# aharley/pips

Hardware: AMD Instinct MI355X
Metric: particle-updates/sec (B*S*N*iters/s) at S=8 N=256 368x496 (higher is better)
Workload: dtype f32; 1 GPU; BASELINE configs[1]: B=1/GPU S=8 368x496 N=256 I=6 fp32 stride 8, encoder included, inputs resident in HBM; clips_per_gpu=1, parallelism=clip-sharded x1, collective=none

## Files before the change

pips_amd/csrc/conv_f32_r.hip:

```cpp
#include "common.h"

namespace pips {

constexpr int CR_ROWS = 4, CR_COLS = 32, CR_TN = 32, CR_PITCH = 272;
constexpr int CR_PW = CR_COLS + 2, CR_PH = CR_ROWS + 2;
constexpr int CR_WBYTES = 9 * CR_TN * CR_PITCH, CR_PBYTES = CR_PH * CR_PW * CR_PITCH;
constexpr int CR_LDS = CR_WBYTES + CR_PBYTES;
constexpr int CR_NCH = CR_PH * CR_PW * 16, CR_NIT = (CR_NCH + 255) / 256;
constexpr unsigned CR_OOB = 0x80000000u;

struct ConvRArgs {
    const float* in; const float* wgt; const float* bias; float* out; float* stats; const float* in_norm;
    int H, W, tiles_x, tiles, bph;
    int by_xcd;
};

typedef unsigned u32x4 __attribute__((ext_vector_type(4)));

__global__ __launch_bounds__(256) void conv3x3_c64_f32_r_kernel(ConvRArgs p) {
    extern __shared__ __attribute__((aligned(16))) char smem[];
    char* Wl = smem;
    char* Pl = smem + CR_WBYTES;
    const int tid = threadIdx.x, lane = tid & 63;
    const int wave = __builtin_amdgcn_readfirstlane(tid >> 6);
    const int l31 = lane & 31, half = lane >> 5;
    const int H = p.H, W = p.W;
    int f, rem;
    if (p.by_xcd) {
        const int per = 16 * p.bph, grp = blockIdx.x / per, j = blockIdx.x - grp * per;
        f = 8 * grp + (j & 7); rem = j >> 3;
    } else {
        f = blockIdx.x / (2 * p.bph); rem = blockIdx.x - f * (2 * p.bph);
    }
    const int hc = rem & 1, b = rem >> 1;

    {
        constexpr int NW = 9 * CR_TN * 16 / 256;
        float4 wv[NW];
#pragma unroll
        for (int k = 0; k < NW; ++k) {
            const int i = tid + 256 * k, row = i >> 4, tap = row >> 5, co = row & 31;
            wv[k] = *reinterpret_cast<const float4*>(p.wgt + ((size_t)(hc * CR_TN + co) * 9 + tap) * 64 + (i & 15) * 4);
        }
#pragma unroll
        for (int k = 0; k < NW; ++k) {
            const int i = tid + 256 * k;
            *reinterpret_cast<float4*>(Wl + (i >> 4) * CR_PITCH + (i & 15) * 16) = wv[k];
        }
    }

    const __amdgpu_buffer_rsrc_t rsrc = __builtin_amdgcn_make_buffer_rsrc(
        const_cast<float*>(p.in + (size_t)f * H * W * 64), (short)0, (int)((unsigned)(H * W) * 256u), 0x00020000);
    const int chunk = tid & 15;
    unsigned goff[CR_NIT], pyx[CR_NIT];
#pragma unroll
    for (int it = 0; it < CR_NIT; ++it) {
        const int pix = (tid >> 4) + it * 16;
        const int py = pix / CR_PW, px = pix - py * CR_PW;
        goff[it] = (unsigned)((py * W + px) * 256 + chunk * 16);
        pyx[it] = (unsigned)(py | px << 8);
    }
    const bool last_ok = tid + (CR_NIT - 1) * 256 < CR_NCH;
    char* lds_dst = Pl + (tid >> 4) * CR_PITCH + chunk * 16;
    float4 nrm[2] = {make_float4(0.f, 1.f, 0.f, 1.f), make_float4(0.f, 1.f, 0.f, 1.f)};
    if (p.in_norm != nullptr) {
        const float4* np = reinterpret_cast<const float4*>(p.in_norm + ((size_t)f * 64 + chunk * 4) * 2);
        nrm[0] = np[0]; nrm[1] = np[1];
    }

    u32x4 fr[CR_NIT];
    unsigned inside = 0;
    auto fetch = [&](int t, bool live) __attribute__((always_inline)) {
        const int ty = t / p.tiles_x, tx = t - ty * p.tiles_x;
        const int y0 = ty * CR_ROWS, x0 = tx * CR_COLS;
        const unsigned base = (unsigned)(((y0 - 1) * W + (x0 - 1)) * 256);
        const bool interior = y0 >= 1 && y0 + CR_ROWS + 1 <= H && x0 >= 1 && x0 + CR_COLS + 1 <= W;
        if (interior) {
            inside = last_ok ? (1u << CR_NIT) - 1 : (1u << (CR_NIT - 1)) - 1;
#pragma unroll
            for (int it = 0; it < CR_NIT; ++it) {
                const unsigned off = (live && (it + 1 < CR_NIT || last_ok)) ? base + goff[it] : CR_OOB;
                fr[it] = __builtin_amdgcn_raw_buffer_load_b128(rsrc, (int)off, 0, 0);
            }
        } else {
            inside = 0;
#pragma unroll
            for (int it = 0; it < CR_NIT; ++it) {
                const int gy = y0 - 1 + (int)(pyx[it] & 0xff), gx = x0 - 1 + (int)(pyx[it] >> 8);
                const bool ok = live && (it + 1 < CR_NIT || last_ok) && (unsigned)gy < (unsigned)H && (unsigned)gx < (unsigned)W;
                inside |= ok ? 1u << it : 0u;
                fr[it] = __builtin_amdgcn_raw_buffer_load_b128(rsrc, (int)(ok ? base + goff[it] : CR_OOB), 0, 0);
            }
        }
    };
    auto stage = [&]() __attribute__((always_inline)) {
#pragma unroll
        for (int it = 0; it < CR_NIT; ++it) {
            if (it + 1 < CR_NIT || last_ok) {
                float4 v = make_float4(__uint_as_float(fr[it].x), __uint_as_float(fr[it].y), __uint_as_float(fr[it].z),
                                       __uint_as_float(fr[it].w));
                if (p.in_norm != nullptr) {
                    const bool in = inside >> it & 1;
                    const float nx = fmaxf((v.x - nrm[0].x) * nrm[0].y, 0.f), ny = fmaxf((v.y - nrm[0].z) * nrm[0].w, 0.f);
                    const float nz = fmaxf((v.z - nrm[1].x) * nrm[1].y, 0.f), nw = fmaxf((v.w - nrm[1].z) * nrm[1].w, 0.f);
                    v = make_float4(in ? nx : 0.f, in ? ny : 0.f, in ? nz : 0.f, in ? nw : 0.f);
                }
                *reinterpret_cast<float4*>(lds_dst + it * (16 * CR_PITCH)) = v;
            }
        }
    };

    const int col = hc * CR_TN + l31;
    const float bv = p.bias[col];
    const char* pa = Pl + (wave * CR_PW + l31) * CR_PITCH + half * 16;
    const char* pb = Wl + l31 * CR_PITCH + half * 16;
    const int parts = p.tiles * 4;
    const __amdgpu_buffer_rsrc_t rsrc_out = __builtin_amdgcn_make_buffer_rsrc(
        p.out + (size_t)f * H * W * 64, (short)0, (int)((unsigned)(H * W) * 256u), 0x00020000);
    const __amdgpu_buffer_rsrc_t rsrc_st = __builtin_amdgcn_make_buffer_rsrc(
        p.stats + (size_t)f * parts * 256, (short)0, (int)((unsigned)parts * 1024u), 0x00020000);

    float bvs = bv;
    asm volatile("" : "+v"(bvs), "+v"(nrm[0].x), "+v"(nrm[0].y), "+v"(nrm[0].z), "+v"(nrm[0].w), "+v"(nrm[1].x), "+v"(nrm[1].y),
                 "+v"(nrm[1].z), "+v"(nrm[1].w));
    fetch(b, true);
#pragma unroll
    for (int r = 0; r < 16; ++r) __builtin_amdgcn_raw_buffer_store_b32((unsigned)r, rsrc_out, (int)(CR_OOB + 256u * r), 0, 0);
    __builtin_amdgcn_raw_buffer_store_b128((u32x4){0u, 0u, 0u, 0u}, rsrc_st, (int)CR_OOB, 0, 0);
    for (int t = b; t < p.tiles; t += p.bph) {
        lds_barrier();
        stage();
        lds_barrier();
        fetch(t + p.bph < p.tiles ? t + p.bph : t, t + p.bph < p.tiles);
        __builtin_amdgcn_sched_barrier(0);

        f32x16 acc;
#pragma unroll
        for (int r = 0; r < 16; ++r) acc[r] = 0.f;
        constexpr int CR_AHEAD = 2, CR_NBUF = 3;
        float4 fa[CR_NBUF], fb[CR_NBUF];
#define PIPS_CR_LOAD(g_)                                                                                                \
        {                                                                                                               \
            constexpr int tap_ = (g_) / 8, kb_ = (g_) % 8, kh_ = tap_ / 3, kw_ = tap_ % 3, buf_ = (g_) % CR_NBUF;         \
            fa[buf_] = *reinterpret_cast<const float4*>(pa + (kh_ * CR_PW + kw_) * CR_PITCH + kb_ * 32);                 \
            fb[buf_] = *reinterpret_cast<const float4*>(pb + tap_ * (CR_TN * CR_PITCH) + kb_ * 32);                      \
        }
#define PIPS_CR_STEP(g_)                                                                                                \
        if constexpr ((g_) + CR_AHEAD < 72) PIPS_CR_LOAD((g_) + CR_AHEAD)                                               \
        acc = __builtin_amdgcn_mfma_f32_32x32x2f32(fa[(g_) % CR_NBUF].x, fb[(g_) % CR_NBUF].x, acc, 0, 0, 0);            \
        acc = __builtin_amdgcn_mfma_f32_32x32x2f32(fa[(g_) % CR_NBUF].y, fb[(g_) % CR_NBUF].y, acc, 0, 0, 0);            \
        acc = __builtin_amdgcn_mfma_f32_32x32x2f32(fa[(g_) % CR_NBUF].z, fb[(g_) % CR_NBUF].z, acc, 0, 0, 0);            \
        acc = __builtin_amdgcn_mfma_f32_32x32x2f32(fa[(g_) % CR_NBUF].w, fb[(g_) % CR_NBUF].w, acc, 0, 0, 0);            \
        __builtin_amdgcn_sched_barrier(0);
#define PIPS_CR_STEP8(g_)                                                                                               \
        PIPS_CR_STEP(g_) PIPS_CR_STEP((g_) + 1) PIPS_CR_STEP((g_) + 2) PIPS_CR_STEP((g_) + 3) PIPS_CR_STEP((g_) + 4)      \
        PIPS_CR_STEP((g_) + 5) PIPS_CR_STEP((g_) + 6) PIPS_CR_STEP((g_) + 7)
        PIPS_CR_LOAD(0) PIPS_CR_LOAD(1)
        __builtin_amdgcn_sched_barrier(0);
        PIPS_CR_STEP8(0) PIPS_CR_STEP8(8) PIPS_CR_STEP8(16) PIPS_CR_STEP8(24) PIPS_CR_STEP8(32) PIPS_CR_STEP8(40) PIPS_CR_STEP8(48)
        PIPS_CR_STEP8(56) PIPS_CR_STEP8(64)
#undef PIPS_CR_STEP8
#undef PIPS_CR_STEP
#undef PIPS_CR_LOAD

        const int ty = t / p.tiles_x, tx = t - ty * p.tiles_x;
        const int y = ty * CR_ROWS + wave, x0 = tx * CR_COLS;
        const int nvalid = y < H ? min(CR_COLS, W - x0) : 0;
        const unsigned obase = (unsigned)(((y * W + x0) * 64 + col) * 4);
        const float piv1 = __shfl(acc[1] + bvs, l31), piv0 = __shfl(acc[0] + bvs, l31);
        const float pivot = nvalid > 1 ? piv1 : piv0;
        float cs = 0.f, cq = 0.f;
#pragma unroll
        for (int r = 0; r < 16; ++r) {
            const int px = (r & 3) + 8 * (r >> 2) + 4 * half;
            const float v = acc[r] + bvs;
            const bool ok = px < nvalid;
            __builtin_amdgcn_raw_buffer_store_b32(__float_as_uint(v), rsrc_out, (int)(ok ? obase + (unsigned)px * 256u : CR_OOB), 0, 0);
            const float d = ok ? v - pivot : 0.f;
            cs += d;
            cq += d * d;
        }
        const float s1 = cs + __shfl_xor(cs, 32), s2 = cq + __shfl_xor(cq, 32);
        const u32x4 sv = {__float_as_uint(s1), __float_as_uint(s2), __float_as_uint(pivot), __float_as_uint((float)nvalid)};
        __builtin_amdgcn_raw_buffer_store_b128(sv, rsrc_st, (int)(half == 0 ? (unsigned)(((t * 4 + wave) * 64 + col) * 16) : CR_OOB), 0, 0);
    }
}

bool conv_f32_r_admits(const GemmArgs& a) {
    if (a.KH != 3 || a.KW != 3 || a.cstride != 1 || a.pad != 1 || a.Cin != 64 || a.N != 64 || a.ldc != 64 || a.Ho != a.H ||
        a.Wo != a.Win || a.bias == nullptr || a.stats == nullptr)
        return false;
    if ((unsigned long long)(a.H + 2) * (a.Win + 2) * 256ull >= (1ull << 31)) return false;
    const long parts = 4l * cdiv(a.H, CR_ROWS) * cdiv(a.Win, CR_COLS);
    const long cap = a.stats_parts_cap > 0 ? a.stats_parts_cap : 2 * cdiv(a.M, 64) + 4;
    return parts <= cap && parts * 64 * 16 < (1l << 31);
}

bool conv_f32_r_takes(const GemmArgs& a, int frames) {
    if (!PIPS_TUNE("PIPS_CONV_F32_R", 1) || !conv_f32_r_admits(a)) return false;
    const int cus = device_cus();
    const long tiles = 2l * cdiv(a.H, CR_ROWS) * cdiv(a.Win, CR_COLS) * frames;
    return cus > 0 && tiles * 100 >= (long)cus * PIPS_TUNE("PIPS_CONV_F32_R_MINPCT", 300);
}

int launch_conv_f32_r(const GemmArgs& a, int frames, int* parts_out, hipStream_t st) {
    const int cus = device_cus();
    if (cus <= 0) {
        set_error("conv3x3_c64_f32_r: cannot query the device");
        return PIPS_E_LAUNCH;
    }
    static std::atomic<unsigned long long> raised{0};
    const int rc = ensure_dynamic_lds(raised, (const void*)conv3x3_c64_f32_r_kernel, CR_LDS);
    if (rc != PIPS_OK) return rc;
    ConvRArgs p;
    p.in = a.A; p.wgt = a.W; p.bias = a.bias; p.out = a.C; p.stats = a.stats; p.in_norm = a.in_norm;
    p.H = a.H; p.W = a.Win; p.tiles_x = cdiv(a.Win, CR_COLS); p.tiles = p.tiles_x * cdiv(a.H, CR_ROWS);
    p.bph = max(1, min(p.tiles, cdiv(cus, 2 * frames)));
    p.by_xcd = (frames % 8 == 0) && PIPS_TUNE("PIPS_CONV_F32_R_XCD", 1);
    hipLaunchKernelGGL(conv3x3_c64_f32_r_kernel, dim3(frames * 2 * p.bph), dim3(256), CR_LDS, st, p);
    PIPS_CHECK_LAUNCH("conv3x3_c64_f32_r_kernel");
    if (parts_out) *parts_out = p.tiles * 4;
    return PIPS_OK;
}

}
```

Baseline: 1.410 million particle-updates/s.

## Compute two 4-row halves per weight fetch with XOR-swizzled unpadded LDS

The 3x3 conv tile grows from 4 to up to 8 output rows per work item. Each wave now keeps two MFMA accumulators that share the same weight fragment loads, so B-operand LDS traffic per output drops. The padded LDS pitch is replaced by an XOR swizzle on 16-byte chunks to avoid bank conflicts. Next-tile global loads are interleaved into the MFMA k-loop instead of being issued in one burst, and work is split into contiguous unit ranges per block. The staging path gets specialized normalization variants. An optional timing trace is compiled in only under a macro. The trade-offs are higher register pressure from the doubled accumulators and more index bookkeeping.

Result: no change. 1.409 million particle-updates/s (-0.1%).

```diff
diff --git a/pips_amd/csrc/conv_f32_r.hip b/pips_amd/csrc/conv_f32_r.hip
--- a/pips_amd/csrc/conv_f32_r.hip
+++ b/pips_amd/csrc/conv_f32_r.hip
@@ -1,26 +1,78 @@
+#include <type_traits>
+
 #include "common.h"
 
 namespace pips {
 
-constexpr int CR_ROWS = 4, CR_COLS = 32, CR_TN = 32, CR_PITCH = 272;
-constexpr int CR_PW = CR_COLS + 2, CR_PH = CR_ROWS + 2;
-constexpr int CR_WBYTES = 9 * CR_TN * CR_PITCH, CR_PBYTES = CR_PH * CR_PW * CR_PITCH;
+constexpr int CR_HROWS = 4, CR_COLS = 32, CR_TN = 32, CR_ROWB = 256;
+constexpr int CR_PW = CR_COLS + 2, CR_PH = 2 * CR_HROWS + 2;
+constexpr int CR_WBYTES = 9 * CR_TN * CR_ROWB, CR_PBYTES = CR_PH * CR_PW * CR_ROWB;
 constexpr int CR_LDS = CR_WBYTES + CR_PBYTES;
 constexpr int CR_NCH = CR_PH * CR_PW * 16, CR_NIT = (CR_NCH + 255) / 256;
 constexpr unsigned CR_OOB = 0x80000000u;
+static_assert(CR_LDS <= 163840, "conv3x3_c64_f32_r: weights and patch must fit the compute unit's LDS");
 
 struct ConvRArgs {
     const float* in; const float* wgt; const float* bias; float* out; float* stats; const float* in_norm;
-    int H, W, tiles_x, tiles, bph;
+    int H, W, tiles_x, rows4;
+    int units, ufull, bph;
     int by_xcd;
 };
 
 typedef unsigned u32x4 __attribute__((ext_vector_type(4)));
 
+#ifdef PIPS_CONV_R_TRACE
+__device__ unsigned long long* g_cr_trace = nullptr;
+#define PIPS_CR_T(i_)                                                        \
+    {                                                                        \
+        __builtin_amdgcn_sched_barrier(0);                                   \
+        const unsigned long long now_ = __builtin_amdgcn_s_memtime();        \
+        tr_acc[i_] += now_ - tr_last;                                        \
+        tr_last = now_;                                                      \
+        __builtin_amdgcn_sched_barrier(0);                                   \
+    }
+#else
+#define PIPS_CR_T(i_)
+#endif
+
+template <int NCH>
+__device__ __forceinline__ void cr_kloop(const char* smem, const unsigned (&pa)[3][8], const unsigned (&pb)[8], f32x16& acc0, f32x16& acc1,
+                                         const __amdgpu_buffer_rsrc_t rsrc, const unsigned (&poff)[CR_NIT], u32x4 (&fr)[CR_NIT]) {
+    static_assert(3 * (CR_NIT - 1) + 1 < 72, "conv3x3_c64_f32_r: one prefetch load per third group");
+    constexpr int CR_AHEAD = 2, CR_NBUF = 3;
+    float4 fa0[CR_NBUF], fa1[CR_NBUF], fb[CR_NBUF];
+#define PIPS_CR_LOAD(g_)                                                                                                \
+    {                                                                                                                   \
+        constexpr int tap_ = (g_) / 8, kb_ = (g_) % 8, kh_ = tap_ / 3, kw_ = tap_ % 3, buf_ = (g_) % CR_NBUF;             \
+        fa0[buf_] = *reinterpret_cast<const float4*>(smem + (pa[kw_][kb_] + kh_ * (CR_PW * CR_ROWB)));                   \
+        if constexpr (NCH == 2)                                                                                         \
+            fa1[buf_] = *reinterpret_cast<const float4*>(smem + (pa[kw_][kb_] + (kh_ + CR_HROWS) * (CR_PW * CR_ROWB)));  \
+        fb[buf_] = *reinterpret_cast<const float4*>(smem + (pb[kb_] + tap_ * (CR_TN * CR_ROWB)));                        \
+    }
+#define PIPS_CR_MFMA(g_, c_)                                                                                            \
+    acc0 = __builtin_amdgcn_mfma_f32_32x32x2f32(fa0[(g_) % CR_NBUF].c_, fb[(g_) % CR_NBUF].c_, acc0, 0, 0, 0);           \
+    if constexpr (NCH == 2) acc1 = __builtin_amdgcn_mfma_f32_32x32x2f32(fa1[(g_) % CR_NBUF].c_, fb[(g_) % CR_NBUF].c_, acc1, 0, 0, 0);
+#define PIPS_CR_STEP(g_)                                                                                                \
+    if constexpr ((g_) % 3 == 1 && (g_) / 3 < CR_NIT)                                                                   \
+        fr[(g_) / 3] = __builtin_amdgcn_raw_buffer_load_b128(rsrc, (int)poff[(g_) / 3], 0, 0);                           \
+    if constexpr ((g_) + CR_AHEAD < 72) PIPS_CR_LOAD((g_) + CR_AHEAD)                                                   \
+    PIPS_CR_MFMA(g_, x) PIPS_CR_MFMA(g_, y) PIPS_CR_MFMA(g_, z) PIPS_CR_MFMA(g_, w)                                      \
+    __builtin_amdgcn_sched_barrier(0);
+#define PIPS_CR_STEP8(g_)                                                                                               \
+    PIPS_CR_STEP(g_) PIPS_CR_STEP((g_) + 1) PIPS_CR_STEP((g_) + 2) PIPS_CR_STEP((g_) + 3) PIPS_CR_STEP((g_) + 4)          \
+    PIPS_CR_STEP((g_) + 5) PIPS_CR_STEP((g_) + 6) PIPS_CR_STEP((g_) + 7)
+    PIPS_CR_LOAD(0) PIPS_CR_LOAD(1)
+    __builtin_amdgcn_sched_barrier(0);
+    PIPS_CR_STEP8(0) PIPS_CR_STEP8(8) PIPS_CR_STEP8(16) PIPS_CR_STEP8(24) PIPS_CR_STEP8(32) PIPS_CR_STEP8(40) PIPS_CR_STEP8(48)
+    PIPS_CR_STEP8(56) PIPS_CR_STEP8(64)
+#undef PIPS_CR_STEP8
+#undef PIPS_CR_STEP
+#undef PIPS_CR_MFMA
+#undef PIPS_CR_LOAD
+}
+
 __global__ __launch_bounds__(256) void conv3x3_c64_f32_r_kernel(ConvRArgs p) {
     extern __shared__ __attribute__((aligned(16))) char smem[];
-    char* Wl = smem;
-    char* Pl = smem + CR_WBYTES;
     const int tid = threadIdx.x, lane = tid & 63;
     const int wave = __builtin_amdgcn_readfirstlane(tid >> 6);
     const int l31 = lane & 31, half = lane >> 5;
@@ -33,6 +85,7 @@
         f = blockIdx.x / (2 * p.bph); rem = blockIdx.x - f * (2 * p.bph);
     }
     const int hc = rem & 1, b = rem >> 1;
+    const int u0 = (int)((long)b * p.units / p.bph), u1 = (int)((long)(b + 1) * p.units / p.bph);
 
     {
         constexpr int NW = 9 * CR_TN * 16 / 256;
@@ -44,77 +97,97 @@
         }
 #pragma unroll
         for (int k = 0; k < NW; ++k) {
-            const int i = tid + 256 * k;
-            *reinterpret_cast<float4*>(Wl + (i >> 4) * CR_PITCH + (i & 15) * 16) = wv[k];
+            const int i = tid + 256 * k, row = i >> 4;
+            *reinterpret_cast<float4*>(smem + row * CR_ROWB + (((i ^ row) & 15) << 4)) = wv[k];
         }
     }
 
     const __amdgpu_buffer_rsrc_t rsrc = __builtin_amdgcn_make_buffer_rsrc(
         const_cast<float*>(p.in + (size_t)f * H * W * 64), (short)0, (int)((unsigned)(H * W) * 256u), 0x00020000);
     const int chunk = tid & 15;
-    unsigned goff[CR_NIT], pyx[CR_NIT];
+    unsigned goff[CR_NIT], ldst[CR_NIT];
 #pragma unroll
     for (int it = 0; it < CR_NIT; ++it) {
         const int pix = (tid >> 4) + it * 16;
         const int py = pix / CR_PW, px = pix - py * CR_PW;
         goff[it] = (unsigned)((py * W + px) * 256 + chunk * 16);
-        pyx[it] = (unsigned)(py | px << 8);
+        ldst[it] = (unsigned)(CR_WBYTES + pix * CR_ROWB + (((chunk ^ px) & 15) << 4));
     }
     const bool last_ok = tid + (CR_NIT - 1) * 256 < CR_NCH;
-    char* lds_dst = Pl + (tid >> 4) * CR_PITCH + chunk * 16;
     float4 nrm[2] = {make_float4(0.f, 1.f, 0.f, 1.f), make_float4(0.f, 1.f, 0.f, 1.f)};
     if (p.in_norm != nullptr) {
         const float4* np = reinterpret_cast<const float4*>(p.in_norm + ((size_t)f * 64 + chunk * 4) * 2);
         nrm[0] = np[0]; nrm[1] = np[1];
     }
 
+    auto halves = [&](int u, int ty, int hh) __attribute__((always_inline)) { return (hh == 0 && 2 * ty + 1 < p.rows4 && u + 2 <= u1) ? 2 : 1; };
+    auto advance = [&](int& u, int& ty, int& tx, int& hh, int nh) __attribute__((always_inline)) {
+        u += nh;
+        if (2 * ty + 1 >= p.rows4) ++tx;
+        else if ((hh += nh) >= 2) { hh = 0; ++tx; }
+        if (tx == p.tiles_x) { tx = 0; ++ty; }
+    };
+
     u32x4 fr[CR_NIT];
+    unsigned poff[CR_NIT];
     unsigned inside = 0;
-    auto fetch = [&](int t, bool live) __attribute__((always_inline)) {
-        const int ty = t / p.tiles_x, tx = t - ty * p.tiles_x;
-        const int y0 = ty * CR_ROWS, x0 = tx * CR_COLS;
+    auto plan = [&](int y0, int x0, int nh, bool live) __attribute__((always_inline)) {
         const unsigned base = (unsigned)(((y0 - 1) * W + (x0 - 1)) * 256);
-        const bool interior = y0 >= 1 && y0 + CR_ROWS + 1 <= H && x0 >= 1 && x0 + CR_COLS + 1 <= W;
+        const bool interior = live && nh == 2 && y0 >= 1 && y0 + 2 * CR_HROWS + 1 <= H && x0 >= 1 && x0 + CR_COLS + 1 <= W;
         if (interior) {
             inside = last_ok ? (1u << CR_NIT) - 1 : (1u << (CR_NIT - 1)) - 1;
 #pragma unroll
-            for (int it = 0; it < CR_NIT; ++it) {
-                const unsigned off = (live && (it + 1 < CR_NIT || last_ok)) ? base + goff[it] : CR_OOB;
-                fr[it] = __builtin_amdgcn_raw_buffer_load_b128(rsrc, (int)off, 0, 0);
-            }
+            for (int it = 0; it < CR_NIT; ++it) poff[it] = (it + 1 < CR_NIT || last_ok) ? base + goff[it] : CR_OOB;
         } else {
             inside = 0;
+            int tq = tid >> 4;
+            asm volatile("" : "+v"(tq));
+            const int prows = nh * CR_HROWS + 2;
 #pragma unroll
             for (int it = 0; it < CR_NIT; ++it) {
-                const int gy = y0 - 1 + (int)(pyx[it] & 0xff), gx = x0 - 1 + (int)(pyx[it] >> 8);
-                const bool ok = live && (it + 1 < CR_NIT || last_ok) && (unsigned)gy < (unsigned)H && (unsigned)gx < (unsigned)W;
+                const int pix = tq + it * 16, py = pix / CR_PW, px = pix - py * CR_PW;
+                const int gy = y0 - 1 + py, gx = x0 - 1 + px;
+                const bool ok = live && (it + 1 < CR_NIT || last_ok) && py < prows && (unsigned)gy < (unsigned)H && (unsigned)gx < (unsigned)W;
                 inside |= ok ? 1u << it : 0u;
-                fr[it] = __builtin_amdgcn_raw_buffer_load_b128(rsrc, (int)(ok ? base + goff[it] : CR_OOB), 0, 0);
+                poff[it] = ok ? base + goff[it] : CR_OOB;
             }
         }
+        return interior;
     };
-    auto stage = [&]() __attribute__((always_inline)) {
+    auto stage_as = [&](auto mode) __attribute__((always_inline)) {
+        constexpr int MODE = decltype(mode)::value;
 #pragma unroll
         for (int it = 0; it < CR_NIT; ++it) {
             if (it + 1 < CR_NIT || last_ok) {
                 float4 v = make_float4(__uint_as_float(fr[it].x), __uint_as_float(fr[it].y), __uint_as_float(fr[it].z),
                                        __uint_as_float(fr[it].w));
-                if (p.in_norm != nullptr) {
-                    const bool in = inside >> it & 1;
+                if constexpr (MODE != 0) {
                     const float nx = fmaxf((v.x - nrm[0].x) * nrm[0].y, 0.f), ny = fmaxf((v.y - nrm[0].z) * nrm[0].w, 0.f);
                     const float nz = fmaxf((v.z - nrm[1].x) * nrm[1].y, 0.f), nw = fmaxf((v.w - nrm[1].z) * nrm[1].w, 0.f);
+                    const bool in = MODE == 1 || (inside >> it & 1);
                     v = make_float4(in ? nx : 0.f, in ? ny : 0.f, in ? nz : 0.f, in ? nw : 0.f);
                 }
-                *reinterpret_cast<float4*>(lds_dst + it * (16 * CR_PITCH)) = v;
+                *reinterpret_cast<float4*>(smem + ldst[it]) = v;
             }
         }
+    };
+    auto stage = [&](bool interior) __attribute__((always_inline)) {
+        if (p.in_norm == nullptr) stage_as(std::integral_constant<int, 0>{});
+        else if (interior) stage_as(std::integral_constant<int, 1>{});
+        else stage_as(std::integral_constant<int, 2>{});
     };
 
     const int col = hc * CR_TN + l31;
     const float bv = p.bias[col];
-    const char* pa = Pl + (wave * CR_PW + l31) * CR_PITCH + half * 16;
-    const char* pb = Wl + l31 * CR_PITCH + half * 16;
-    const int parts = p.tiles * 4;
+    unsigned pa[3][8], pb[8];
+#pragma unroll
+    for (int kb = 0; kb < 8; ++kb) {
+#pragma unroll
+        for (int kw = 0; kw < 3; ++kw)
+            pa[kw][kb] = (unsigned)(CR_WBYTES + (wave * CR_PW + l31 + kw) * CR_ROWB + (((2 * kb + half) ^ (l31 + kw)) & 15) * 16);
+        pb[kb] = (unsigned)(l31 * CR_ROWB + (((2 * kb + half) ^ l31) & 15) * 16);
+    }
+    const int parts = p.rows4 * p.tiles_x * 4;
     const __amdgpu_buffer_rsrc_t rsrc_out = __builtin_amdgcn_make_buffer_rsrc(
         p.out + (size_t)f * H * W * 64, (short)0, (int)((unsigned)(H * W) * 256u), 0x00020000);
     const __amdgpu_buffer_rsrc_t rsrc_st = __builtin_amdgcn_make_buffer_rsrc(
@@ -123,75 +196,95 @@
     float bvs = bv;
     asm volatile("" : "+v"(bvs), "+v"(nrm[0].x), "+v"(nrm[0].y), "+v"(nrm[0].z), "+v"(nrm[0].w), "+v"(nrm[1].x), "+v"(nrm[1].y),
                  "+v"(nrm[1].z), "+v"(nrm[1].w));
-    fetch(b, true);
-#pragma unroll
-    for (int r = 0; r < 16; ++r) __builtin_amdgcn_raw_buffer_store_b32((unsigned)r, rsrc_out, (int)(CR_OOB + 256u * r), 0, 0);
-    __builtin_amdgcn_raw_buffer_store_b128((u32x4){0u, 0u, 0u, 0u}, rsrc_st, (int)CR_OOB, 0, 0);
-    for (int t = b; t < p.tiles; t += p.bph) {
+    int u = u0, ty, tx, hh;
+    if (u0 < p.ufull) {
+        const int t8 = u0 >> 1;
+        hh = u0 & 1; ty = t8 / p.tiles_x; tx = t8 - ty * p.tiles_x;
+    } else {
+        hh = 0; ty = p.rows4 >> 1; tx = u0 - p.ufull;
+    }
+    int nh = halves(u, ty, hh);
+    bool interior = plan((2 * ty + hh) * CR_HROWS, tx * CR_COLS, nh, true);
+#pragma unroll
+    for (int it = 0; it < CR_NIT; ++it) fr[it] = __builtin_amdgcn_raw_buffer_load_b128(rsrc, (int)poff[it], 0, 0);
+#pragma unroll
+    for (int c = 0; c < 2; ++c) {
+#pragma unroll
+        for (int r = 0; r < 16; ++r)
+            __builtin_amdgcn_raw_buffer_store_b32((unsigned)(16 * c + r), rsrc_out, (int)(CR_OOB + 256u * (16 * c + r)), 0, 0);
+        __builtin_amdgcn_raw_buffer_store_b128((u32x4){0u, 0u, 0u, 0u}, rsrc_st, (int)(CR_OOB + 16u * c), 0, 0);
+    }
+#ifdef PIPS_CONV_R_TRACE
+    unsigned long long tr_acc[8] = {0, 0, 0, 0, 0, 0, 0, 0}, tr_last = __builtin_amdgcn_s_memtime();
+    unsigned tr_items = 0, tr_halves = 0;
+#endif
+    while (u < u1) {
+        PIPS_CR_T(0)
         lds_barrier();
-        stage();
+        PIPS_CR_T(1)
+        stage(interior);
+        PIPS_CR_T(2)
         lds_barrier();
-        fetch(t + p.bph < p.tiles ? t + p.bph : t, t + p.bph < p.tiles);
+        PIPS_CR_T(3)
+        int un = u, tyn = ty, txn = tx, hhn = hh;
+        advance(un, tyn, txn, hhn, nh);
+        const int nn = un < u1 ? halves(un, tyn, hhn) : 1;
+        interior = plan((2 * tyn + hhn) * CR_HROWS, txn * CR_COLS, nn, un < u1);
         __builtin_amdgcn_sched_barrier(0);
-
-        f32x16 acc;
-#pragma unroll
-        for (int r = 0; r < 16; ++r) acc[r] = 0.f;
-        constexpr int CR_AHEAD = 2, CR_NBUF = 3;
-        float4 fa[CR_NBUF], fb[CR_NBUF];
-#define PIPS_CR_LOAD(g_)                                                                                                \
-        {                                                                                                               \
-            constexpr int tap_ = (g_) / 8, kb_ = (g_) % 8, kh_ = tap_ / 3, kw_ = tap_ % 3, buf_ = (g_) % CR_NBUF;         \
-            fa[buf_] = *reinterpret_cast<const float4*>(pa + (kh_ * CR_PW + kw_) * CR_PITCH + kb_ * 32);                 \
-            fb[buf_] = *reinterpret_cast<const float4*>(pb + tap_ * (CR_TN * CR_PITCH) + kb_ * 32);                      \
-        }
-#define PIPS_CR_STEP(g_)                                                                                                \
-        if constexpr ((g_) + CR_AHEAD < 72) PIPS_CR_LOAD((g_) + CR_AHEAD)                                               \
-        acc = __builtin_amdgcn_mfma_f32_32x32x2f32(fa[(g_) % CR_NBUF].x, fb[(g_) % CR_NBUF].x, acc, 0, 0, 0);            \
-        acc = __builtin_amdgcn_mfma_f32_32x32x2f32(fa[(g_) % CR_NBUF].y, fb[(g_) % CR_NBUF].y, acc, 0, 0, 0);            \
-        acc = __builtin_amdgcn_mfma_f32_32x32x2f32(fa[(g_) % CR_NBUF].z, fb[(g_) % CR_NBUF].z, acc, 0, 0, 0);            \
-        acc = __builtin_amdgcn_mfma_f32_32x32x2f32(fa[(g_) % CR_NBUF].w, fb[(g_) % CR_NBUF].w, acc, 0, 0, 0);            \
-        __builtin_amdgcn_sched_barrier(0);
-#define PIPS_CR_STEP8(g_)                                                                                               \
-        PIPS_CR_STEP(g_) PIPS_CR_STEP((g_) + 1) PIPS_CR_STEP((g_) + 2) PIPS_CR_STEP((g_) + 3) PIPS_CR_STEP((g_) + 4)      \
-        PIPS_CR_STEP((g_) + 5) PIPS_CR_STEP((g_) + 6) PIPS_CR_STEP((g_) + 7)
-        PIPS_CR_LOAD(0) PIPS_CR_LOAD(1)
-        __builtin_amdgcn_sched_barrier(0);
-        PIPS_CR_STEP8(0) PIPS_CR_STEP8(8) PIPS_CR_STEP8(16) PIPS_CR_STEP8(24) PIPS_CR_STEP8(32) PIPS_CR_STEP8(40) PIPS_CR_STEP8(48)
-        PIPS_CR_STEP8(56) PIPS_CR_STEP8(64)
-#undef PIPS_CR_STEP8
-#undef PIPS_CR_STEP
-#undef PIPS_CR_LOAD
-
-        const int ty = t / p.tiles_x, tx = t - ty * p.tiles_x;
-        const int y = ty * CR_ROWS + wave, x0 = tx * CR_COLS;
-        const int nvalid = y < H ? min(CR_COLS, W - x0) : 0;
-        const unsigned obase = (unsigned)(((y * W + x0) * 64 + col) * 4);
-        const float piv1 = __shfl(acc[1] + bvs, l31), piv0 = __shfl(acc[0] + bvs, l31);
-        const float pivot = nvalid > 1 ? piv1 : piv0;
-        float cs = 0.f, cq = 0.f;
-#pragma unroll
-        for (int r = 0; r < 16; ++r) {
-            const int px = (r & 3) + 8 * (r >> 2) + 4 * half;
-            const float v = acc[r] + bvs;
-            const bool ok = px < nvalid;
-            __builtin_amdgcn_raw_buffer_store_b32(__float_as_uint(v), rsrc_out, (int)(ok ? obase + (unsigned)px * 256u : CR_OOB), 0, 0);
-            const float d = ok ? v - pivot : 0.f;
-            cs += d;
-            cq += d * d;
-        }
-        const float s1 = cs + __shfl_xor(cs, 32), s2 = cq + __shfl_xor(cq, 32);
-        const u32x4 sv = {__float_as_uint(s1), __float_as_uint(s2), __float_as_uint(pivot), __float_as_uint((float)nvalid)};
-        __builtin_amdgcn_raw_buffer_store_b128(sv, rsrc_st, (int)(half == 0 ? (unsigned)(((t * 4 + wave) * 64 + col) * 16) : CR_OOB), 0, 0);
-    }
+        PIPS_CR_T(4)
+
+        f32x16 acc[2];
+#pragma unroll
+        for (int r = 0; r < 16; ++r) acc[0][r] = acc[1][r] = 0.f;
+        if (nh == 2) cr_kloop<2>(smem, pa, pb, acc[0], acc[1], rsrc, poff, fr);
+        else cr_kloop<1>(smem, pa, pb, acc[0], acc[1], rsrc, poff, fr);
+        PIPS_CR_T(5)
+
+        const int y0 = (2 * ty + hh) * CR_HROWS, x0 = tx * CR_COLS;
+#pragma unroll
+        for (int c = 0; c < 2; ++c) {
+            const int y = y0 + wave + c * CR_HROWS;
+            const bool run = c < nh;
+            const int nvalid = run && y < H ? min(CR_COLS, W - x0) : 0;
+            const unsigned obase = (unsigned)(((y * W + x0) * 64 + col) * 4);
+            const float piv1 = __shfl(acc[c][1] + bvs, l31), piv0 = __shfl(acc[c][0] + bvs, l31);
+            const float pivot = nvalid > 1 ? piv1 : piv0;
+            float cs = 0.f, cq = 0.f;
+#pragma unroll
+            for (int r = 0; r < 16; ++r) {
+                const int px = (r & 3) + 8 * (r >> 2) + 4 * half;
+                const float v = acc[c][r] + bvs;
+                const bool ok = px < nvalid;
+                __builtin_amdgcn_raw_buffer_store_b32(__float_as_uint(v), rsrc_out, (int)(ok ? obase + (unsigned)px * 256u : CR_OOB), 0, 0);
+                const float d = ok ? v - pivot : 0.f;
+                cs += d;
+                cq += d * d;
+            }
+            const float s1 = cs + __shfl_xor(cs, 32), s2 = cq + __shfl_xor(cq, 32);
+            const u32x4 sv = {__float_as_uint(s1), __float_as_uint(s2), __float_as_uint(pivot), __float_as_uint((float)nvalid)};
+            const unsigned slot = (unsigned)(((y >> 2) * p.tiles_x + tx) * 4 + (y & 3));
+            __builtin_amdgcn_raw_buffer_store_b128(sv, rsrc_st, (int)(half == 0 && run ? (slot * 64 + col) * 16 : CR_OOB), 0, 0);
+        }
+#ifdef PIPS_CONV_R_TRACE
+        ++tr_items; tr_halves += nh == 1;
+#endif
+        u = un; ty = tyn; tx = txn; hh = hhn; nh = nn;
+    }
+#ifdef PIPS_CONV_R_TRACE
+    if (tid == 0 && g_cr_trace != nullptr) {
+        unsigned long long* o = g_cr_trace + (size_t)blockIdx.x * 10;
+        for (int i = 0; i < 8; ++i) o[i] = tr_acc[i];
+        o[8] = tr_items; o[9] = tr_halves;
+    }
+#endif
 }
 
 bool conv_f32_r_admits(const GemmArgs& a) {
     if (a.KH != 3 || a.KW != 3 || a.cstride != 1 || a.pad != 1 || a.Cin != 64 || a.N != 64 || a.ldc != 64 || a.Ho != a.H ||
         a.Wo != a.Win || a.bias == nullptr || a.stats == nullptr)
         return false;
-    if ((unsigned long long)(a.H + 2) * (a.Win + 2) * 256ull >= (1ull << 31)) return false;
-    const long parts = 4l * cdiv(a.H, CR_ROWS) * cdiv(a.Win, CR_COLS);
+    if ((unsigned long long)(a.H + 2 * CR_HROWS + 2) * (a.Win + CR_COLS + 2) * 256ull >= (1ull << 31)) return false;
+    const long parts = 4l * cdiv(a.H, CR_HROWS) * cdiv(a.Win, CR_COLS);
     const long cap = a.stats_parts_cap > 0 ? a.stats_parts_cap : 2 * cdiv(a.M, 64) + 4;
     return parts <= cap && parts * 64 * 16 < (1l << 31);
 }
@@ -199,7 +292,7 @@
 bool conv_f32_r_takes(const GemmArgs& a, int frames) {
     if (!PIPS_TUNE("PIPS_CONV_F32_R", 1) || !conv_f32_r_admits(a)) return false;
     const int cus = device_cus();
-    const long tiles = 2l * cdiv(a.H, CR_ROWS) * cdiv(a.Win, CR_COLS) * frames;
+    const long tiles = 2l * cdiv(a.H, CR_HROWS) * cdiv(a.Win, CR_COLS) * frames;
     return cus > 0 && tiles * 100 >= (long)cus * PIPS_TUNE("PIPS_CONV_F32_R_MINPCT", 300);
 }
 
@@ -214,13 +307,20 @@
     if (rc != PIPS_OK) return rc;
     ConvRArgs p;
     p.in = a.A; p.wgt = a.W; p.bias = a.bias; p.out = a.C; p.stats = a.stats; p.in_norm = a.in_norm;
-    p.H = a.H; p.W = a.Win; p.tiles_x = cdiv(a.Win, CR_COLS); p.tiles = p.tiles_x * cdiv(a.H, CR_ROWS);
-    p.bph = max(1, min(p.tiles, cdiv(cus, 2 * frames)));
+    p.H = a.H; p.W = a.Win; p.tiles_x = cdiv(a.Win, CR_COLS); p.rows4 = cdiv(a.H, CR_HROWS);
+    p.units = p.tiles_x * p.rows4; p.ufull = 2 * p.tiles_x * (p.rows4 / 2);
+    p.bph = max(1, min(p.units, cdiv(cus, 2 * frames)));
     p.by_xcd = (frames % 8 == 0) && PIPS_TUNE("PIPS_CONV_F32_R_XCD", 1);
     hipLaunchKernelGGL(conv3x3_c64_f32_r_kernel, dim3(frames * 2 * p.bph), dim3(256), CR_LDS, st, p);
     PIPS_CHECK_LAUNCH("conv3x3_c64_f32_r_kernel");
-    if (parts_out) *parts_out = p.tiles * 4;
+    if (parts_out) *parts_out = p.units * 4;
     return PIPS_OK;
 }
 
 }
+
+#ifdef PIPS_CONV_R_TRACE
+extern "C" int pips_conv_r_trace(void* buf) {
+    return hipMemcpyToSymbol(HIP_SYMBOL(pips::g_cr_trace), &buf, sizeof(buf)) == hipSuccess ? 0 : -3;
+}
+#endif
```
